# UCD4IDS/WaveletsExt.jl

Hardware: AMD Instinct MI355X
Metric: Msamples/s (fwd+inv wavelet packets) (higher is better)
Workload: dtype f64

## Files before the change

### waveletsext.jl_amd/__init__.py

```python
from .filters import WT, OrthoFilter, ArgumentError, wavelet, daubechies
from .util import (maxtransformlevels, isdyadic, ndyadicscales, nodelength, getchildindex,
                   getparentindex, getdepth, gettreelength, maketree, isvalidtree, getleaf,
                   getrowrange, getcolrange, main2depthshift, coarsestscalingrange,
                   finestdetailrange, delete_subtree)
from ._arrays import jl_empty, to_device, to_numpy, to_colmajor
from ._lib import WxError, build_info, device_count, red2d_route, set_force_generic, set_host_hugepages, shutdown, LIB_PATH
from .dwt import (wpd, wpd_, wpdall, iwpd, iwpd_, iwpdall, wpt, wpt_, iwpt, iwpt_,
                  wptall, iwptall, getbasiscoef, getbasiscoefall, dwt, idwt, dwtall, idwtall)
from .swt import (sdwt, sdwt_, sdwtall, isdwt, isdwt_, isdwtall, swpt, swpt_, swptall, iswpt, iswpt_,
                  iswptall, swpd, swpd_, swpdall, iswpd, iswpd_, iswpdall)
from .acwt import (acdwt, acdwt_, acdwtall, iacdwt, iacdwt_, iacdwtall, acwpt, acwpt_, acwptall,
                   iacwpt, iacwpt_, iacwptall, acwpd, acwpd_, acwpdall, iacwpd, iacwpd_, iacwpdall,
                   autocorr, pfilter, qfilter, make_acqmfpair, make_acreverseqmfpair)
from .bestbasis import (JBB, LoglpCost, NormCost, tree_costs, bestbasistree, bestbasis_treeselection,
                        jbb_moments, costs_from_moments, acwpd_jbb_moments,
                        BB, ShannonEntropyCost, LogEnergyEntropyCost, bestbasistreeall,
                        LSDB, DifferentialEntropyCost, lsdb_entropy)
from .denoising import (HardTH, SoftTH, SemiSoftTH, SteinTH, VisuShrink, SureShrink, RelErrorShrink,
                        noisest, threshold, denoise, denoiseall, surethreshold, relerrorthreshold,
                        surethresholdall, relerrorthresholdall)
from .ldb import (TimeFrequency, AsymmetricRelativeEntropy, SymmetricRelativeEntropy, LpDistance,
                  HellingerDistance, EarthMoverDistance, ProbabilityDensity, Signatures, SignatureMap, BasisDiscriminantMeasure,
                  FishersClassSeparability, RobustFishersClassSeparability, energy_map,
                  discriminant_measure, discriminant_power, LocalDiscriminantBasis, fit_, fitdec_, transform,
                  fit_transform, inverse_transform, change_nfeatures)
from .siwt import (ShiftInvariantWaveletTransformNode, ShiftInvariantWaveletTransformObject,
                   ShiftInvariantWaveletTransformBatch, siwpd, siwpdall, isiwpd, isiwpdall, bestbasistree_,
                   bestbasistreeall_, delete_node_)
from . import siwt as _siwt
_isvalidtree_arrays = isvalidtree


def isvalidtree(*args, **kw):
    if len(args) == 1 and isinstance(args[0], ShiftInvariantWaveletTransformObject):
        return _siwt.isvalidtree(args[0], **kw)
    return _isvalidtree_arrays(*args, **kw)
```

### waveletsext.jl_amd/_lib.py

```python
import ctypes
import os

_HERE = os.path.dirname(os.path.abspath(__file__))
LIB_PATH = os.environ.get("WX_HIP_LIB") or os.path.join(_HERE, "csrc", "libwaveletsext_hip.so")

WX_OK, WX_EASSERT, WX_EARG, WX_EBOUNDS, WX_EHIP, WX_EUNSUPPORTED = 0, -1, -2, -3, -10, -11


class WxError(RuntimeError):
    def __init__(self, code, msg):
        super().__init__("libwaveletsext_hip status %d: %s" % (code, msg))
        self.code = code


_lib = None


def lib():
    global _lib
    if _lib is None:
        if not os.path.exists(LIB_PATH):
            raise ImportError(
                "libwaveletsext_hip.so is not built (%s). Run `python -c 'import __graft_entry__ as g; "
                "g.build()'` or `make -C waveletsext.jl_amd/csrc`. There is no CPU fallback." % LIB_PATH)
# ... 97 lines not shown
    "wx_class_median_mad_f64": [_P, _L, _L, _P, _I, _P, _P, _P],
    "wx_class_median_mad_f32": [_P, _L, _L, _P, _I, _P, _P, _P],
    "wx_emd_measure_f64": [_P, _L, _L, _P, _I, _P, _P],
    "wx_emd_measure_f32": [_P, _L, _L, _P, _I, _P, _P],
    "wx_pdf_energy_map_f64": [_P, _L, _L, _P, _I, _P, _P],
    "wx_pdf_energy_map_f32": [_P, _L, _L, _P, _I, _P, _P],
    "wx_signature_weights_f64": [_P, _L, _L, _P, _I, _P, _P],
    "wx_signature_weights_f32": [_P, _L, _L, _P, _I, _P, _P],
    "wx_emd_measure_weighted_f64": [_P, _P, _L, _L, _P, _I, _P, _P],
    "wx_emd_measure_weighted_f32": [_P, _P, _L, _L, _P, _I, _P, _P],
    "wx_noisest_f64": [_P, _L, _L, _L, _L, _L, _P, _P],
    "wx_noisest_f32": [_P, _L, _L, _L, _L, _L, _P, _P],
    "wx_threshold_f64": [_P, _P, _L, _L, _L, _I, _P, _L, _L, _P, _P],
    "wx_threshold_f32": [_P, _P, _L, _L, _L, _I, _P, _L, _L, _P, _P],
    "wx_dwt3d_f64": [_P, _P, _L, _L, _L, _I, _L, _P, _I, _P],
    "wx_dwt3d_f32": [_P, _P, _L, _L, _L, _I, _L, _P, _I, _P],
    "wx_idwt3d_f64": [_P, _P, _L, _L, _L, _I, _L, _P, _I, _P],
    "wx_idwt3d_f32": [_P, _P, _L, _L, _L, _I, _L, _P, _I, _P],
    "wx_denoiseall_dwt_f64": [_P, _P, _L, _I, _L, _P, _I, _I, ctypes.c_double, _I, _P, _P],
    "wx_denoiseall_dwt_f32": [_P, _P, _L, _I, _L, _P, _I, _I, ctypes.c_double, _I, _P, _P],
    "wx_denoiseall_sig_f64": [_P, _P, _L, _I, _L, _P, _I, _I, ctypes.c_double, _I, _P, _P],
    "wx_denoiseall_sig_f32": [_P, _P, _L, _I, _L, _P, _I, _I, ctypes.c_double, _I, _P, _P],
    "wx_iwpt1d_thresh_f64": [_P, _P, _L, _I, _P, _L, _L, _P, _I, _I, _P, _L, _L, ctypes.c_double, _P],
    "wx_iwpt1d_thresh_f32": [_P, _P, _L, _I, _P, _L, _L, _P, _I, _I, _P, _L, _L, ctypes.c_double, _P],
    "wx_surethreshold_f64": [_P, _L, _L, _L, _P, _P, _P],
    "wx_surethreshold_f32": [_P, _L, _L, _L, _P, _P, _P],
    "wx_relerrorthreshold_f64": [_P, _L, _L, _L, _P, _I, _P, _P],
    "wx_relerrorthreshold_f32": [_P, _L, _L, _L, _P, _I, _P, _P],
    "wx_bb_costs_f64": [_P, _P, _L, _L, _L, _I, _I, _P],
    "wx_bb_costs_f32": [_P, _P, _L, _L, _L, _I, _I, _P],
    "wx_bb_costs2d_f64": [_P, _P, _L, _L, _L, _L, _I, _I, _P],
    "wx_bb_costs2d_f32": [_P, _P, _L, _L, _L, _L, _I, _I, _P],
    "wx_lsdb_entropy_f64": [_P, _L, _L, _P, _P],
    "wx_lsdb_entropy_f32": [_P, _L, _L, _P, _P],
    "wx_lsdb_costs_f64": [_P, _L, _L, _L, _I, _P, _P],
    "wx_lsdb_costs_f32": [_P, _L, _L, _L, _I, _P, _P],
    "wx_lsdb_costs2d_f64": [_P, _L, _L, _L, _L, _I, _P, _P],
    "wx_lsdb_costs2d_f32": [_P, _L, _L, _L, _L, _I, _P, _P],
    "wx_treeselect_batch_f64": [_P, _L, _L, _L, _I, _L, _P, _P],
    "wx_treeselect_batch_f32": [_P, _L, _L, _L, _I, _L, _P, _P],
    "wx_comm_unique_id": [_P],
    "wx_comm_init": [_I, _I, _P, ctypes.POINTER(ctypes.c_void_p)],
    "wx_comm_destroy": [_P],
    "wx_allgather_out_f64": [_P, _P, _L, _P, _P],
    "wx_allgather_out_f32": [_P, _P, _L, _P, _P],
    "wx_allgatherv_out_f64": [_P, _P, _P, _I, _P, _P],
    "wx_allgatherv_out_f32": [_P, _P, _P, _I, _P, _P],
    "wx_allreduce_moments_f64": [_P, _L, _P, _P],
    "wx_allreduce_moments_f32": [_P, _L, _P, _P],
}


def check(rc):
    if rc == WX_OK:
        return
    msg = lib().wx_last_error().decode("utf-8", "replace")
    if rc == WX_EASSERT:
        raise AssertionError(msg)
    if rc == WX_EARG:
        from .filters import ArgumentError
        raise ArgumentError(msg)
    if rc == WX_EBOUNDS:
        raise IndexError(msg)
    raise WxError(rc, msg)


def device_count():
    return lib().wx_device_count()


def build_info():
    return lib().wx_build_info().decode("utf-8", "replace")


def shutdown():
    check(lib().wx_shutdown())


def set_host_hugepages(on):
    return bool(lib().wx_set_host_hugepages(1 if on else 0))


def set_force_generic(on):
    lib().wx_debug_set_dispatch(2 if on == 2 else (1 if on else 0))


RED2D_ROUTES = {1: "F1", 2: "F2", 3: "F3", 4: "I1", 5: "I2", 6: "I3", 7: "I4"}


def red2d_route(inverse, m, n, L, elem_size, F, ac=False, shift=False):
    code = lib().wx_debug_red2d_route(int(bool(inverse)), m, n, L, elem_size, F, int(bool(ac)), int(bool(shift)))
    if code < 0:
        raise ValueError("wx_debug_red2d_route: arguments outside the transforms' domain")
    return RED2D_ROUTES[code & 255], code >> 8
```

### waveletsext.jl_amd/csrc/wx_api.hip

```cpp
#include "../../include/waveletsext_hip.h"
#include "wx_host.h"
#include "wx_debug.h"
#include "wx_kernels.h"
#include "wx_lanetree.h"
#include "wx_lattice_dn_api.h"
#include <atomic>
#include <cstring>

const char *wx_err_cstr();
static std::atomic<int> g_force_generic{0};
int wx_force_generic() { return g_force_generic.load() == 1; }
int wx_skip_register_kernels() { return g_force_generic.load() == 2; }

extern "C" {

int wx_version(void) { return 100;  }
const char *wx_last_error(void) { return wx_err_cstr(); }
int wx_device_count(void)
{
    int n = 0;
    if (hipGetDeviceCount(&n) != hipSuccess) { (void)hipGetLastError(); return 0; }
    return n;
}
void wx_debug_set_dispatch(int on) { g_force_generic.store(on == 2 ? 2 : (on ? 1 : 0)); }

}

#define WX_REQUIRE(cond, code, msg) \
    do { if (!(cond)) return wx_set_error(code, msg); } while (0)

static int wx_need_device()
{
    if (wx_device_count() < 1) return wx_set_error(WX_EHIP, "no HIP device visible: the MI355X kernels cannot run");
    return WX_OK;
}

template <typename T>
static int api_wpd1d(const T *x, T *y, int64_t n, int L, int64_t batch, const double *qmf, int F, void *stream)
{
    WxFilt filt;
    int rc = wx_pack_filter(qmf, F, &filt);
    if (rc) return rc;
    WX_REQUIRE(n >= 1 && batch >= 0, WX_EARG, "wpd: bad dimensions");
    WX_REQUIRE(0 <= L && L <= wx_maxtransformlevels(n), WX_EASSERT, "wpd!: 0 <= L <= maxtransformlevels(x) (DWT.jl:137)");
    WX_REQUIRE(n < ((int64_t)1 << 30), WX_EUNSUPPORTED, "wpd: signal length >= 2^30 not supported");
    if ((rc = wx_need_device())) return rc;
    hipStream_t st = wx_stream(stream);
    WxIO io(st);
    const T *dx = (const T *)io.in(x, sizeof(T) * n * batch);
    T *dy = (T *)io.out(y, sizeof(T) * n * (L + 1) * batch);
    if ((batch && n) && (!dx || !dy)) return io.finish(WX_EHIP);
    rc = wx_dev_wpd1d<T>(dx, dy, n, L, batch, filt, st, wx_force_generic());
    return io.finish(rc);
}

struct WxTree1d {
    int Leff = 0;
    const uint8_t *dstatus = nullptr;
    int64_t nstatus = 0;
    bool full = true;
};

static int wx_resolve_tree1d(int64_t n, int L, const uint8_t *tree, int64_t ntree, WxScratch &scr, WxTree1d *out,
                             const char *who)
{
    (void)who;
    WX_REQUIRE(wx_isdyadic(n), WX_EASSERT, "maketree/isvalidtree: signal length must be dyadic (Wavelets.jl)");
    if (!tree) {
        WX_REQUIRE(0 <= L && L <= wx_maxtransformlevels(n), WX_EASSERT, "maketree: 0 <= L <= maxtransformlevels(n)");
        out->Leff = L;
        out->full = true;
        return WX_OK;
    }
    WX_REQUIRE(wx_isvalidtree1d(n, tree, ntree), WX_EASSERT, "@assert isvalidtree(x, tree)");
    out->Leff = wx_tree_depth1d(tree, ntree);
    bool full = true;
    for (int64_t i = 1; i <= ((int64_t)1 << out->Leff) - 1 && full; ++i) full = tree[i - 1] != 0;
    out->full = full;
    if (!full) {
        out->dstatus = (const uint8_t *)scr.upload(tree, (size_t)ntree);
        if (!out->dstatus) return WX_EHIP;
        out->nstatus = ntree;
    }
    return WX_OK;
}

template <typename T>
static int wx_pyramid_tail(int64_t n, int F, bool inverse, const uint8_t *tree, int64_t ntree, std::vector<uint8_t> &cut, const WxFilt &filt,
                           bool allow_long = false)
{
    if (!tree || wx_force_generic()) return 0;
    const int Ld = wx_tree_depth1d(tree, ntree);
    bool pyramid = Ld >= 1;
    for (int64_t i = 1; i <= ntree && pyramid; ++i) pyramid = (tree[i - 1] != 0) == ((i & (i - 1)) == 0 && i < ((int64_t)1 << Ld));
    if (!pyramid) return 0;
    const int tail = wx_dwt_tail_levels(n, Ld, F, sizeof(T));
    if (!tail || (inverse && !((wx_fused1d_ok<T>(n, F) || (allow_long && wx_dwt_long_ok<T>(n, filt))) && Ld - tail >= 2))) return 0;
    cut.assign(tree, tree + ntree);
    for (int64_t i = (int64_t)1 << (Ld - tail); i <= ntree; ++i) cut[i - 1] = 0;
    return tail;
}

template <typename T, bool INVERSE>
static int api_wpt1d(const T *x, T *y, int64_t n, int L, const uint8_t *tree, int64_t ntree, int64_t batch,
                     const double *qmf, int F, void *stream)
{
    WxFilt filt;
// ... 368 lines not shown
```

### waveletsext.jl_amd/csrc/wx_debug.h

```cpp
#pragma once
#include <stdint.h>
#ifdef __cplusplus
extern "C" {
#endif
void wx_debug_set_dispatch(int mode);

int wx_debug_red2d_route(int inverse, int64_t m, int64_t n, int L, int elem_size, int F, int ac, int shift);
#ifdef __cplusplus
}
#endif
```

### waveletsext.jl_amd/csrc/wx_lattice.hip

```cpp
#include "wx_lattice_dev.h"

bool wx_lattice_factor(const WxFilt &filt, int L, bool inverse, WxLat *out)
{
    const int F = filt.F;
    if (F < 2 || (F & 1) || F / 2 > WX_LAT_MAXS) return false;
    const int J = F / 2 - 1;
    long double G[WX_LAT_MAXS][2][2] = {};
    for (int m = 0; m <= J; ++m) {
        G[m][0][0] = filt.q[2 * m];
        G[m][0][1] = filt.q[2 * m + 1];
        G[J - m][1][0] = -(long double)filt.q[2 * m + 1];
        G[J - m][1][1] = filt.q[2 * m];
    }
    long double t[WX_LAT_MAXS], cs[WX_LAT_MAXS];
    for (int deg = J; deg >= 1; --deg) {
        const int k = (fabsl(G[deg][0][0]) + fabsl(G[deg][1][0]) >= fabsl(G[deg][0][1]) + fabsl(G[deg][1][1])) ? 0 : 1;
        const long double a0 = G[deg][0][k], a1 = G[deg][1][k], r = hypotl(a0, a1);
        if (!(r > 0)) return false;
        const long double c = a1 / r, s = a0 / r;
        long double Hm[WX_LAT_MAXS][2][2];
        for (int m = 0; m <= deg; ++m)
            for (int col = 0; col < 2; ++col) {
                Hm[m][0][col] = c * G[m][0][col] - s * G[m][1][col];
                Hm[m][1][col] = s * G[m][0][col] + c * G[m][1][col];
            }
        for (int col = 0; col < 2; ++col)
            if (fabsl(Hm[deg][0][col]) > 1e-13L || fabsl(Hm[0][1][col]) > 1e-13L) return false;
        for (int m = 0; m < deg; ++m)
            for (int col = 0; col < 2; ++col) {
                G[m][0][col] = Hm[m][0][col];
                G[m][1][col] = Hm[m + 1][1][col];
            }
        if (fabsl(c) < 1e-3L) return false;
        t[deg] = s / c;
        cs[deg] = c;
    }
    {
        const long double c = G[0][0][0], s = G[0][0][1];
        if (fabsl(G[0][1][0] + s) > 1e-13L || fabsl(G[0][1][1] - c) > 1e-13L || fabsl(c) < 1e-3L) return false;
        t[0] = s / c;
        cs[0] = c;
    }
    long double gain1 = 1;
    double tr[WX_LAT_MAXS];
    for (int j = 0; j <= J; ++j) {
        tr[j] = (double)t[j];
        gain1 *= cs[j];
    }
    long double P[WX_LAT_MAXS][2][2] = {};
    P[0][0][0] = 1; P[0][0][1] = tr[0]; P[0][1][0] = -(long double)tr[0]; P[0][1][1] = 1;
    for (int j = 1; j <= J; ++j) {
        long double Q[WX_LAT_MAXS][2][2] = {};
        const long double tj = tr[j];
        for (int m = 0; m < j; ++m)
            for (int col = 0; col < 2; ++col) {
                Q[m][0][col] += P[m][0][col];
                Q[m + 1][0][col] += tj * P[m][1][col];
                Q[m][1][col] += -tj * P[m][0][col];
                Q[m + 1][1][col] += P[m][1][col];
            }
        for (int m = 0; m <= j; ++m)
            for (int r2 = 0; r2 < 2; ++r2)
                for (int col = 0; col < 2; ++col) P[m][r2][col] = Q[m][r2][col];
    }
    for (int m = 0; m <= J; ++m)
        if (fabsl(gain1 * P[m][0][0] - filt.q[2 * m]) > 1e-14L || fabsl(gain1 * P[m][0][1] - filt.q[2 * m + 1]) > 1e-14L)
            return false;
    long double sig = 1;
    for (int j = 0; j < WX_LAT_MAXS; ++j) {
        if (j <= J) {
            const long double c2 = 1 / (1 + t[j] * t[j]);
            out->p[j] = (double)(t[j] / sig);
            out->kap[j] = (double)(sig * t[j] * c2);
            sig *= c2;
        } else {
            out->p[j] = out->kap[j] = 0.0;
        }
    }
    const long double gL = powl(gain1, L);
    out->g0 = (double)(inverse ? 1 / gL : gL);
    out->g2 = (double)(inverse ? gain1 * gain1 : 1 / (gain1 * gain1));
    return std::isfinite(out->g0) && fabsl(gL) > 1e-60L && fabsl(gL) < 1e60L;
}

bool wx_lattice_coeffs(const WxFilt &filt, int L, bool inverse, double *p, double *kap, double *g0, double *g2)
{
    WxLat c;
    if (!wx_lattice_factor(filt, L, inverse, &c)) return false;
    for (int j = 0; j < WX_LAT_MAXS; ++j) { p[j] = c.p[j]; kap[j] = c.kap[j]; }
    *g0 = c.g0;
    *g2 = c.g2;
    return true;
}

int wx_lattice_launch_sh(bool inverse, const double *x, double *y, int64_t n, int L, int64_t batch, int64_t in_stride,
                         const WxFilt &filt, hipStream_t st);
int wx_lattice_launch_g(bool inverse, const double *x, double *y, int64_t n, int L, int64_t batch, int64_t in_stride,
                        const WxFilt &filt, hipStream_t st);
int wx_lattice_wpd_g_f64(const double *x, double *y, int64_t n, int L, int64_t batch, const WxFilt &filt, hipStream_t st);
int wx_lattice_launch_lo(bool inverse, const double *x, double *y, int L, int64_t batch, int64_t in_stride, const WxFilt &filt,
                         hipStream_t st);

static int wx_lattice_launch(bool inverse, const double *x, double *y, int64_t n, int L, int64_t batch, int64_t in_stride,
                             const WxFilt &filt, hipStream_t st)
{
    if (n == 2048 || n == 1024)
        return wx_lattice_launch_sh(inverse, x, y, n, L, batch, inverse ? in_stride : n, filt, st);
    if (n >= 64 && n <= 512)
        return wx_lattice_launch_g(inverse, x, y, n, L, batch, inverse ? in_stride : n, filt, st);
    if (n == 4096 && L >= 1 && L <= 5) return wx_lattice_launch_lo(inverse, x, y, L, batch, inverse ? in_stride : n, filt, st);
    if (n != 4096 || L < 6 || L > 12 || filt.F < 2 || batch <= 0) return 0;
    if ((reinterpret_cast<uintptr_t>(x) | reinterpret_cast<uintptr_t>(y)) & 31) return 0;
    if (inverse && (in_stride & 3)) return 0;
    WxLat cf;
    if (!wx_lattice_factor(filt, L, inverse, &cf)) return 0;
    int64_t grid = batch;
    if (grid > 0x7fffffff) grid = 0x7fffffff;
#define WX_GO(NSS)                                                                                                  \
    case NSS:                                                                                                       \
        if (inverse)                                                                                                \
            hipLaunchKernelGGL((k_lat_iwpt_f64<NSS, 2>), dim3((unsigned)grid), dim3(64), 0, st, x, y, L, batch, in_stride, cf); \
        else                                                                                                        \
            hipLaunchKernelGGL((k_lat_wpt_f64<NSS, 3>), dim3((unsigned)grid), dim3(64), 0, st, x, y, L, batch, cf);  \
        break;
    switch (wx_lat_stages(filt.F)) {
        WX_GO(1) WX_GO(2) WX_GO(4) WX_GO(6) WX_GO(8) WX_GO(10)
    default: return 0;
    }
#undef WX_GO
    const hipError_t e = hipGetLastError();
    if (e != hipSuccess) return wx_set_hip_error(e, "lattice wpt launch", __FILE__, __LINE__);
    return 1;
}

int wx_lattice_wpd_sh_f64(const double *x, double *y, int64_t n, int L, int64_t batch, const WxFilt &filt, hipStream_t st);

int wx_lattice_wpd_f64(const double *x, double *y, int64_t n, int L, int64_t batch, const WxFilt &filt, hipStream_t st)
{
    if ((n == 2048 || n == 1024) && x != (const double *)y) return wx_lattice_wpd_sh_f64(x, y, n, L, batch, filt, st);
    if (n >= 64 && n <= 512 && x != (const double *)y) return wx_lattice_wpd_g_f64(x, y, n, L, batch, filt, st);
    if (n != 4096 || L < 1 || L > 12 || filt.F < 2 || batch <= 0 || batch > 0x7fffffff) return 0;
    if ((reinterpret_cast<uintptr_t>(x) | reinterpret_cast<uintptr_t>(y)) & 31) return 0;
    WxLatW cw;
    if (!wx_lattice_factor(filt, L, false, &cw.c)) return 0;
    {
        const long double g2 = cw.c.g2;
        long double g = 1 / sqrtl(g2);
        WxLat tmp;
        if (!wx_lattice_factor(filt, 1, false, &tmp)) return 0;
        g = tmp.g0;
        long double acc = 1;
        for (int l = 0; l <= 12; ++l) { cw.gl[l] = (double)acc; acc *= g; }
    }
#define WX_GOW(NSS)                                                                                                 \
    case NSS:                                                                                                       \
        hipLaunchKernelGGL((k_lat_wpd_f64<NSS, 2>), dim3((unsigned)batch), dim3(64), 0, st, x, y, L, batch, cw);     \
        break;
    switch (wx_lat_stages(filt.F)) {
        WX_GOW(1) WX_GOW(2) WX_GOW(4) WX_GOW(6) WX_GOW(8) WX_GOW(10)
    default: return 0;
    }
#undef WX_GOW
    const hipError_t e = hipGetLastError();
    if (e != hipSuccess) return wx_set_hip_error(e, "lattice wpd launch", __FILE__, __LINE__);
    return 1;
}

bool wx_lattice_applicable_f64(const WxFilt &filt)
{
    if (filt.F < 2 || filt.F / 2 > WX_LAT_MAXS) return false;
    WxLat tmp;
    return wx_lattice_factor(filt, 6, false, &tmp);
}

int wx_lattice_wpt8k_f64(const double *x, double *y, int L, int64_t batch, const WxFilt &filt, hipStream_t st);
int wx_lattice_iwpt8k_f64(const double *xw, double *y, int L, int64_t batch, int64_t in_stride, const WxFilt &filt, hipStream_t st);

int wx_lattice_wpt_f64(const double *x, double *y, int64_t n, int L, int64_t batch, const WxFilt &filt, hipStream_t st)
{
    if (n == 8192) return wx_lattice_wpt8k_f64(x, y, L, batch, filt, st);
    return wx_lattice_launch(false, x, y, n, L, batch, n, filt, st);
}
int wx_lattice_iwpt_f64(const double *xw, double *y, int64_t n, int L, int64_t batch, int64_t in_stride, const WxFilt &filt,
                        hipStream_t st)
{
    if (n == 8192) return wx_lattice_iwpt8k_f64(xw, y, L, batch, in_stride, filt, st);
    return wx_lattice_launch(true, xw, y, n, L, batch, in_stride, filt, st);
}

#define WX_TREE_DECL(k)                                                                                              \
    int wx_lattice_tree##k##_f64(bool, const double *, double *, int64_t, int, int64_t, int64_t, int64_t, const WxFilt &, \
                                 const uint8_t *, int64_t, const WxThreshArg *, hipStream_t, int64_t);
WX_TREE_DECL(0f) WX_TREE_DECL(0i) WX_TREE_DECL(1f) WX_TREE_DECL(1i) WX_TREE_DECL(2f) WX_TREE_DECL(2i)
#undef WX_TREE_DECL

#define WX_TREES_DECL(k)                                                                                                             \
    int wx_lattice_trees_##k##_f64(const double *, double *, int64_t, int, int64_t, int64_t, int64_t, const WxFilt &, const uint8_t *, int64_t, hipStream_t, int64_t); \
    int wx_lattice_trees_##k##_f32(const float *, float *, int64_t, int, int64_t, int64_t, int64_t, const WxFilt &, const uint8_t *, int64_t, hipStream_t, int64_t);
WX_TREES_DECL(3f) WX_TREES_DECL(3i) WX_TREES_DECL(4f) WX_TREES_DECL(4i) WX_TREES_DECL(5f) WX_TREES_DECL(5i) WX_TREES_DECL(6f) WX_TREES_DECL(6i)
#undef WX_TREES_DECL
// ... 63 lines not shown
```

### waveletsext.jl_amd/csrc/wx_lattice_8ki.hip

```cpp
#include "wx_lattice_8k.h"
bool wx_lattice_factor(const WxFilt &filt, int L, bool inverse, WxLat *out);
int wx_lattice_iwpt8k_f64(const double *xw, double *y, int L, int64_t batch, int64_t in_stride, const WxFilt &filt, hipStream_t st)
{
    if (L < 7 || L > 13 || filt.F < 2 || filt.F > 20 || batch <= 0 || batch > 0x7fffffff || xw == y) return 0;
    if ((reinterpret_cast<uintptr_t>(xw) | reinterpret_cast<uintptr_t>(y)) & 31) return 0;
    if (in_stride < 8192 || (in_stride & 3)) return 0;
    WxLat cf;
    if (!wx_lattice_factor(filt, L - 1, true, &cf)) return 0;
#define WX_GO8(NSS)                                                                                                      \
    case NSS: hipLaunchKernelGGL((k_lat_iwpt8k_f64<NSS, 2>), dim3((unsigned)batch), dim3(128), 0, st, xw, y, L - 1, batch, in_stride, cf, filt); break;
    switch (wx_lat_stages(filt.F)) {
        WX_GO8(1) WX_GO8(2) WX_GO8(4) WX_GO8(6) WX_GO8(8) WX_GO8(10)
    default: return 0;
    }
#undef WX_GO8
    const hipError_t e = hipGetLastError();
    if (e != hipSuccess) return wx_set_hip_error(e, "lattice iwpt launch (8192 samples)", __FILE__, __LINE__);
    return 1;
}
```

### waveletsext.jl_amd/csrc/wx_lattice_dev.h

```cpp
#pragma once
#include "wx_common.h"
#include "wx_kernels.h"
#include <cmath>
#include <cstdlib>
#include <utility>

#define WX_LAT_MAXS 10
#define WX_LAT_LDS 1104

struct WxLat {
    double p[WX_LAT_MAXS];
    double kap[WX_LAT_MAXS];
    double g0;
    double g2;
};

namespace {

__device__ __forceinline__ void lat_sync()
{
    __builtin_amdgcn_fence(__ATOMIC_RELEASE, "wavefront");
    __builtin_amdgcn_wave_barrier();
    __builtin_amdgcn_fence(__ATOMIC_ACQUIRE, "wavefront");
}
// ... 1011 lines not shown
    lat_level<3, 0, NS, false>(c, cf);
    lat_emit<6, 10>(c, lds0, ys + 4096 * 10, lane, cw);
    if (L < 11) return;
    lat_level<4, 0, NS, false>(c, cf);
    lat_emit<6, 11>(c, lds0, ys + 4096 * 11, lane, cw);
    if (L < 12) return;
    lat_level<5, 0, NS, false>(c, cf);
    lat_emit<6, 12>(c, lds0, ys + 4096 * 12, lane, cw);
}

__device__ __forceinline__ double lat_ld1(const double __attribute__((address_space(1))) *p) { return *p; }
template <int SH> constexpr int lat_rotr(int p) { return (p >> SH) | ((p & ((1 << SH) - 1)) << (12 - SH)); }

template <int NS, int WPE, int SH>
__global__ __launch_bounds__(64) __attribute__((amdgpu_waves_per_eu(WPE, WPE))) void k_lat_wpt_sh_f64(
    const double *__restrict__ x, double *__restrict__ y, int L, int last_sig, WxLatW cw)
{
    static_assert(SH == 1 || SH == 2, "two or four signals per wavefront");
    __shared__ double lds[WX_LAT_LDS];
    const unsigned lds0 = (unsigned)(uintptr_t)(double __attribute__((address_space(3))) *)lds;
    const int lane = threadIdx.x;
    const int sig0 = min((int)blockIdx.x << SH, last_sig);
    const int64_t off = (int64_t)sig0 * (4096 >> SH);
    const double *xs = x + off;
    double *ys = y + off;
    const WxLat &cf = cw.c;
    double a[64];
    {
        lat_d2 r[32];
        const int lp = 64 * (lane >> 3) + 2 * (lane & 7);
        const unsigned xo = (unsigned)((lp >> SH) | ((lp & ((1 << SH) - 1)) << (12 - SH)));
        lat_for<32>([&](auto Q) {
            constexpr int hi3 = Q / 4, f = Q % 4;
            r[Q].x = lat_ld1(lat_sbase(xs + lat_rotr<SH>(512 * hi3 + 16 * f)) + xo);
            r[Q].y = lat_ld1(lat_sbase(xs + lat_rotr<SH>(512 * hi3 + 16 * f + 1)) + xo);
        });
        const unsigned wa = lds0 + 8u * (17u * (lane >> 3) + 2u * (lane & 7)), ra = lds0 + 8u * 17u * lane;
        lat_for<4>([&](auto Fq) {
            constexpr int f = Fq;
            lat_for<8>([&](auto Hq) {
                constexpr int hi3 = Hq;
                lds_wr<8 * (136 * hi3)>(wa, r[4 * hi3 + f].x);
                lds_wr<8 * (136 * hi3 + 1)>(wa, r[4 * hi3 + f].y);
            });
            double t[16];
            lat_for<16>([&](auto M) {
                constexpr int m = M;
                t[m] = lds_rd<8 * m>(ra);
            });
            lat_wait16<0>(t);
            lat_for<16>([&](auto M) {
                constexpr int m = M;
                a[16 * f + m] = t[m];
            });
        });
    }
    if constexpr (SH < 2) lat_level<1, 6, NS, false>(a, cf);
    double bb[64];
    lat_t2(a, bb, lds0, lane);
    lat_level<0, 4, NS, false>(bb, cf);
    lat_level<1, 4, NS, false>(bb, cf);
    lat_level<2, 4, NS, false>(bb, cf);
    lat_level<3, 4, NS, false>(bb, cf);
    double c[64];
    lat_t3(bb, c, lds0, lane);
    const int Le = L + SH;
    if (Le > 6) lat_level<0, 0, NS, false>(c, cf);
    if (Le > 7) lat_level<1, 0, NS, false>(c, cf);
    if (Le > 8) lat_level<2, 0, NS, false>(c, cf);
    if (Le > 9) lat_level<3, 0, NS, false>(c, cf);
    if (Le > 10) lat_level<4, 0, NS, false>(c, cf);
    if (Le > 11) lat_level<5, 0, NS, false>(c, cf);
    switch (Le) {
    case 6: lat_emit<6, 6 - SH + 16 * SH>(c, lds0, ys, lane, cw); break;
    case 7: lat_emit<6, 7 - SH + 16 * SH>(c, lds0, ys, lane, cw); break;
    case 8: lat_emit<6, 8 - SH + 16 * SH>(c, lds0, ys, lane, cw); break;
    case 9: lat_emit<6, 9 - SH + 16 * SH>(c, lds0, ys, lane, cw); break;
    case 10: lat_emit<6, 10 - SH + 16 * SH>(c, lds0, ys, lane, cw); break;
    case 11: lat_emit<6, 11 - SH + 16 * SH>(c, lds0, ys, lane, cw); break;
    default: lat_emit<6, 12 - SH + 16 * SH>(c, lds0, ys, lane, cw); break;
    }
}

template <int NS, typename TM, typename SINK>
__device__ __forceinline__ void lat_inv_to_l0(const TM *__restrict__ xs, unsigned lds0, int lane, int L, const WxLat &cf, SINK &&sink)
{
    double c[64];
    switch (L) {
    case 6: lat_load_c<6>(c, lds0, xs, lane, cf); break;
    case 7: lat_load_c<7>(c, lds0, xs, lane, cf); break;
    case 8: lat_load_c<8>(c, lds0, xs, lane, cf); break;
    case 9: lat_load_c<9>(c, lds0, xs, lane, cf); break;
    case 10: lat_load_c<10>(c, lds0, xs, lane, cf); break;
    case 11: lat_load_c<11>(c, lds0, xs, lane, cf); break;
    default: lat_load_c<12>(c, lds0, xs, lane, cf); break;
    }
    if (L > 11) lat_level<5, 0, NS, true>(c, cf);
    if (L > 10) lat_level<4, 0, NS, true>(c, cf);
    if (L > 9) lat_level<3, 0, NS, true>(c, cf);
    if (L > 8) lat_level<2, 0, NS, true>(c, cf);
    if (L > 7) lat_level<1, 0, NS, true>(c, cf);
    if (L > 6) lat_level<0, 0, NS, true>(c, cf);
    double bb[64];
    {
        const unsigned wa = lds0 + 8u * (34 * (lane >> 1) + (lane & 1));
        const int H = lane & 15, p0 = (lane >> 4) & 1, p1 = lane >> 5;
        const unsigned ra = lds0 + 8u * (34 * p1 + 2 * H + p0);
        lat_for<4>([&](auto Fq) {
            constexpr int f = Fq;
            lat_for<16>([&](auto Hq) {
                constexpr int Hh = Hq;
                lds_wr<8 * 2 * Hh>(wa, c[4 * Hh + f]);
            });
            double t[16];
            lat_for<16>([&](auto Jq) {
                constexpr int j = Jq;
                t[j] = lds_rd<8 * 68 * j>(ra);
            });
            lat_wait16<0>(t);
            lat_for<16>([&](auto Jq) {
                constexpr int j = Jq;
                bb[16 * f + j] = t[j];
            });
        });
    }
    lat_level<3, 4, NS, true>(bb, cf);
    lat_level<2, 4, NS, true>(bb, cf);
    lat_level<1, 4, NS, true>(bb, cf);
    lat_level<0, 4, NS, true>(bb, cf);
    double a[64];
    {
        const int H = lane & 15, p10 = lane >> 4;
        unsigned wa[4];
#pragma unroll
        for (int h = 0; h < 4; ++h)
            wa[h] = lds0 + 8u * (((h ^ (H >> 2)) | ((H & 3) << 2) | (((H >> 2) & 1) << 4) | ((H >> 3) << 5)) + 64 * p10);
        const int Ha = lane >> 2, ha = lane & 3;
        const unsigned ra = lds0 + 8u * ((ha ^ (Ha >> 2)) | ((Ha & 3) << 2) | (((Ha >> 2) & 1) << 4) | ((Ha >> 3) << 5));
        lat_for<4>([&](auto Fq) {
            constexpr int f = Fq;
            lat_for<16>([&](auto Q) {
                constexpr int h = Q / 4, g = Q % 4;
                lds_wr<8 * 256 * g>(wa[h], bb[16 * h + 4 * f + g]);
            });
            double t[16];
            lat_for<16>([&](auto Jq) {
                constexpr int j = Jq;
                t[j] = lds_rd<8 * 64 * j>(ra);
            });
            lat_wait16<0>(t);
            lat_for<16>([&](auto Jq) {
                constexpr int j = Jq;
                a[16 * f + j] = t[j];
            });
        });
    }
    lat_level<1, 6, NS, true>(a, cf);
    lat_level<0, 6, NS, true>(a, cf);
    lat_t1i(a, lds0, lane, sink);
}

template <int NS, int WPE, typename TM = double>
__global__ __launch_bounds__(64) __attribute__((amdgpu_waves_per_eu(WPE, WPE))) void k_lat_iwpt_f64(
    const TM *__restrict__ xw, TM *__restrict__ y, int L, int64_t batch, int64_t in_stride, WxLat cf)
{
    __shared__ double lds[WX_LAT_LDS];
    const unsigned lds0 = (unsigned)(uintptr_t)(double __attribute__((address_space(3))) *)lds;
    const int lane = threadIdx.x;
    const int64_t sig = blockIdx.x;
    const unsigned yo = 64u * (lane >> 3) + 2u * (lane & 7);
    TM *ys = y + sig * 4096;
    lat_inv_to_l0<NS>(xw + sig * in_stride, lds0, lane, L, cf, [&](auto Fq, lat_d2 (&o)[8]) {
        constexpr int f = decltype(Fq)::value;
        lat_for<8>([&](auto Hq) {
            constexpr int hi3 = Hq;
            lat_st2(lat_sbase(ys + 512 * hi3 + 16 * f) + yo, o[hi3]);
        });
    });
}

template <int NS, int WPE, int SH>
__global__ __launch_bounds__(64) __attribute__((amdgpu_waves_per_eu(WPE, WPE))) void k_lat_wpd_sh_f64(
    const double *__restrict__ x, double *__restrict__ y, int L, int last_sig, WxLatW cw)
{
    static_assert(SH == 1 || SH == 2, "two or four signals per wavefront");
    __shared__ double lds[WX_LAT_LDS];
    const unsigned lds0 = (unsigned)(uintptr_t)(double __attribute__((address_space(3))) *)lds;
    const int lane = threadIdx.x;
    constexpr int N = 4096 >> SH;
    const int sig0 = min((int)blockIdx.x << SH, last_sig);
    const double *xs = x + (int64_t)sig0 * N;
    const unsigned ts = (unsigned)(N * (L + 1));
    double *ys = y + (int64_t)sig0 * ts;
    const WxLat &cf = cw.c;
    double a[64];
    {
        lat_d2 r[32];
        const int lp = 64 * (lane >> 3) + 2 * (lane & 7);
        const unsigned xo = (unsigned)((lp >> SH) | ((lp & ((1 << SH) - 1)) << (12 - SH)));
        lat_for<32>([&](auto Q) {
            constexpr int hi3 = Q / 4, f = Q % 4;
            r[Q].x = lat_ld1(lat_sbase(xs + lat_rotr<SH>(512 * hi3 + 16 * f)) + xo);
            r[Q].y = lat_ld1(lat_sbase(xs + lat_rotr<SH>(512 * hi3 + 16 * f + 1)) + xo);
        });
        const unsigned wa = lds0 + 8u * (17u * (lane >> 3) + 2u * (lane & 7)), ra = lds0 + 8u * 17u * lane;
        lat_for<4>([&](auto Fq) {
            constexpr int f = Fq;
            lat_for<8>([&](auto Hq) {
                constexpr int hi3 = Hq;
                lds_wr<8 * (136 * hi3)>(wa, r[4 * hi3 + f].x);
                lds_wr<8 * (136 * hi3 + 1)>(wa, r[4 * hi3 + f].y);
            });
            double t[16];
            lat_for<16>([&](auto M) {
                constexpr int m = M;
                t[m] = lds_rd<8 * m>(ra);
            });
            lat_wait16<0>(t);
            lat_for<16>([&](auto M) {
                constexpr int m = M;
                a[16 * f + m] = t[m];
            });
        });
    }
    lat_emit<0, 16 * SH>(a, lds0, ys, lane, cw, ts);
#define WX_LVL_A(K)                                                                               \
    if constexpr (K >= SH) {                                                                      \
        constexpr int l = K - SH + 1;                                                             \
        lat_level<K, 6, NS, false>(a, cf);                                                        \
        lat_emit<0, l + 16 * SH>(a, lds0, ys + N * l, lane, cw, ts);                              \
        if (L <= l) return;                                                                       \
    }
    WX_LVL_A(1)
#undef WX_LVL_A
    double bb[64];
    lat_t2(a, bb, lds0, lane);
#define WX_LVL_B(K)                                                                               \
    {                                                                                             \
        constexpr int l = K + 2 - SH + 1;                                                         \
        lat_level<K, 4, NS, false>(bb, cf);                                                       \
        lat_emit<2, l + 16 * SH>(bb, lds0, ys + N * l, lane, cw, ts);                             \
        if (L <= l) return;                                                                       \
// ... 407 lines not shown
```

Before: 39610.

## Fold top inverse lattice levels into a dense per-node matrix for L=12

For the inverse wavelet packet lattice at depth 12 (and 13 in the 8192-sample kernel), the host now precomputes a small dense matrix (8x8 or 4x4) that combines the top two or three inverse lattice levels. The kernel applies that matrix to the register-resident coefficients with FMAs instead of running several sequential lattice stages with shifts. This cuts the serial dependency chain and per-stage overhead, but adds NF multiply-adds per output and passes a larger kernel argument. Numerical behaviour changes slightly, and a debug dispatch mode is added to turn the fold off.

```diff
diff --git a/waveletsext.jl_amd/__init__.py b/waveletsext.jl_amd/__init__.py
--- a/waveletsext.jl_amd/__init__.py
+++ b/waveletsext.jl_amd/__init__.py
@@ -4,7 +4,7 @@
                    getrowrange, getcolrange, main2depthshift, coarsestscalingrange,
                    finestdetailrange, delete_subtree)
 from ._arrays import jl_empty, to_device, to_numpy, to_colmajor
-from ._lib import WxError, build_info, device_count, red2d_route, set_force_generic, set_host_hugepages, shutdown, LIB_PATH
+from ._lib import WxError, build_info, device_count, lattice_fold_matrix, red2d_route, set_force_generic, set_host_hugepages, shutdown, LIB_PATH
 from .dwt import (wpd, wpd_, wpdall, iwpd, iwpd_, iwpdall, wpt, wpt_, iwpt, iwpt_,
                   wptall, iwptall, getbasiscoef, getbasiscoefall, dwt, idwt, dwtall, idwtall)
 from .swt import (sdwt, sdwt_, sdwtall, isdwt, isdwt_, isdwtall, swpt, swpt_, swptall, iswpt, iswpt_,
diff --git a/waveletsext.jl_amd/_lib.py b/waveletsext.jl_amd/_lib.py
--- a/waveletsext.jl_amd/_lib.py
+++ b/waveletsext.jl_amd/_lib.py
@@ -203,7 +203,18 @@
 
 
 def set_force_generic(on):
-    lib().wx_debug_set_dispatch(2 if on == 2 else (1 if on else 0))
+    lib().wx_debug_set_dispatch(on if on in (2, 3) else (1 if on else 0))
+
+
+def lattice_fold_matrix(qmf, nf, inverse=True):
+    import numpy as np
+    q = np.ascontiguousarray(qmf, dtype=np.float64)
+    m = np.zeros((nf, nf), dtype=np.float64)
+    f = lib().wx_debug_lattice_fold
+    f.argtypes = [_P, _I, _I, _I, _P]
+    f.restype = _I
+    got = f(q.ctypes.data, int(q.size), int(nf), 1 if inverse else 0, m.ctypes.data)
+    return m if got == nf else None
 
 
 RED2D_ROUTES = {1: "F1", 2: "F2", 3: "F3", 4: "I1", 5: "I2", 6: "I3", 7: "I4"}
diff --git a/waveletsext.jl_amd/csrc/wx_api.hip b/waveletsext.jl_amd/csrc/wx_api.hip
--- a/waveletsext.jl_amd/csrc/wx_api.hip
+++ b/waveletsext.jl_amd/csrc/wx_api.hip
@@ -11,6 +11,7 @@
 static std::atomic<int> g_force_generic{0};
 int wx_force_generic() { return g_force_generic.load() == 1; }
 int wx_skip_register_kernels() { return g_force_generic.load() == 2; }
+int wx_lattice_no_fold() { return g_force_generic.load() == 3; }
 
 extern "C" {
 
@@ -22,7 +23,7 @@
     if (hipGetDeviceCount(&n) != hipSuccess) { (void)hipGetLastError(); return 0; }
     return n;
 }
-void wx_debug_set_dispatch(int on) { g_force_generic.store(on == 2 ? 2 : (on ? 1 : 0)); }
+void wx_debug_set_dispatch(int on) { g_force_generic.store((on == 2 || on == 3) ? on : (on ? 1 : 0)); }
 
 }
 
diff --git a/waveletsext.jl_amd/csrc/wx_debug.h b/waveletsext.jl_amd/csrc/wx_debug.h
--- a/waveletsext.jl_amd/csrc/wx_debug.h
+++ b/waveletsext.jl_amd/csrc/wx_debug.h
@@ -5,6 +5,8 @@
 #endif
 void wx_debug_set_dispatch(int mode);
 
+int wx_debug_lattice_fold(const double *q, int F, int NF, int inverse, double *m);
+
 int wx_debug_red2d_route(int inverse, int64_t m, int64_t n, int L, int elem_size, int F, int ac, int shift);
 #ifdef __cplusplus
 }
diff --git a/waveletsext.jl_amd/csrc/wx_lattice.hip b/waveletsext.jl_amd/csrc/wx_lattice.hip
--- a/waveletsext.jl_amd/csrc/wx_lattice.hip
+++ b/waveletsext.jl_amd/csrc/wx_lattice.hip
@@ -1,4 +1,4 @@
-#include "wx_lattice_dev.h"
+#include "wx_lattice_fold.h"
 
 bool wx_lattice_factor(const WxFilt &filt, int L, bool inverse, WxLat *out)
 {
@@ -83,6 +83,58 @@
     return std::isfinite(out->g0) && fabsl(gL) > 1e-60L && fabsl(gL) < 1e60L;
 }
 
+bool wx_lattice_fold_matrix(const WxLat &cf, int NS, int NF, bool inverse, double *m)
+{
+    if (NS < 1 || NS > WX_LAT_MAXS || (NF != 2 && NF != 4 && NF != 8)) return false;
+    const int nb = NF == 2 ? 1 : (NF == 4 ? 2 : 3);
+    for (int col = 0; col < NF; ++col) {
+        long double x[8] = {};
+        x[col] = 1;
+        for (int k = 0; k < nb; ++k) {
+            const int b = inverse ? nb - 1 - k : k, S = 1 << b, M = NF >> (b + 1);
+            for (int s = 0; s < S; ++s) {
+                long double u[4], w[4], old[4];
+                for (int mm = 0; mm < M; ++mm) { u[mm] = x[s + ((2 * mm) << b)]; w[mm] = x[s + ((2 * mm) << b) + S]; }
+                auto shift = [&](int sh) {
+                    for (int mm = 0; mm < M; ++mm) old[mm] = w[mm];
+                    for (int mm = 0; mm < M; ++mm) w[mm] = old[(((mm + sh) % M) + M) % M];
+                };
+                if (!inverse) {
+                    for (int j = 0; j < NS; ++j) {
+                        for (int mm = 0; mm < M; ++mm) { u[mm] += (long double)cf.p[j] * w[mm]; w[mm] -= (long double)cf.kap[j] * u[mm]; }
+                        if (j + 1 < NS) shift(1);
+                    }
+                    shift(-(NS - 1));
+                } else {
+                    shift(NS - 1);
+                    for (int j = NS - 1; j >= 0; --j) {
+                        for (int mm = 0; mm < M; ++mm) { w[mm] += (long double)cf.kap[j] * u[mm]; u[mm] -= (long double)cf.p[j] * w[mm]; }
+                        if (j > 0) shift(-1);
+                    }
+                }
+                for (int mm = 0; mm < M; ++mm) { x[s + ((2 * mm) << b)] = u[mm]; x[s + ((2 * mm) << b) + S] = w[mm]; }
+            }
+        }
+        for (int i = 0; i < NF; ++i) {
+            if (!std::isfinite((double)x[i]) || fabsl(x[i]) > 1e30L) return false;
+            m[NF * i + col] = (double)x[i];
+        }
+    }
+    return true;
+}
+
+extern "C" int wx_debug_lattice_fold(const double *q, int F, int NF, int inverse, double *m)
+{
+    if (!q || !m || F < 2 || F > WX_MAXF) return 0;
+    WxFilt filt = {};
+    for (int i = 0; i < F; ++i) filt.q[i] = q[i];
+    filt.F = F;
+    WxLat cf;
+    const int NS = wx_lat_stages(F);
+    if (NS < 6 || NS > WX_LAT_MAXS || !wx_lattice_factor(filt, 12, inverse != 0, &cf)) return 0;
+    return wx_lattice_fold_matrix(cf, NS, NF, inverse != 0, m) ? NF : 0;
+}
+
 bool wx_lattice_coeffs(const WxFilt &filt, int L, bool inverse, double *p, double *kap, double *g0, double *g2)
 {
     WxLat c;
@@ -116,6 +168,19 @@
     if (!wx_lattice_factor(filt, L, inverse, &cf)) return 0;
     int64_t grid = batch;
     if (grid > 0x7fffffff) grid = 0x7fffffff;
+    if (inverse && L == 12 && wx_lat_stages(filt.F) >= 6 && !wx_lattice_no_fold()) {
+        WxLatFold<WX_LAT_FOLD> fm;
+        if (wx_lattice_fold_matrix(cf, wx_lat_stages(filt.F), WX_LAT_FOLD, true, fm.m)) {
+            switch (wx_lat_stages(filt.F)) {
+            case 6: hipLaunchKernelGGL((k_lat_iwpt12_f64<6, 2, WX_LAT_FOLD>), dim3((unsigned)grid), dim3(64), 0, st, x, y, batch, in_stride, cf, fm); break;
+            case 8: hipLaunchKernelGGL((k_lat_iwpt12_f64<8, 2, WX_LAT_FOLD>), dim3((unsigned)grid), dim3(64), 0, st, x, y, batch, in_stride, cf, fm); break;
+            default: hipLaunchKernelGGL((k_lat_iwpt12_f64<10, 2, WX_LAT_FOLD>), dim3((unsigned)grid), dim3(64), 0, st, x, y, batch, in_stride, cf, fm); break;
+            }
+            const hipError_t ef = hipGetLastError();
+            if (ef != hipSuccess) return wx_set_hip_error(ef, "lattice iwpt launch (folded)", __FILE__, __LINE__);
+            return 1;
+        }
+    }
 #define WX_GO(NSS)                                                                                                  \
     case NSS:                                                                                                       \
         if (inverse)                                                                                                \
diff --git a/waveletsext.jl_amd/csrc/wx_lattice_8ki.hip b/waveletsext.jl_amd/csrc/wx_lattice_8ki.hip
--- a/waveletsext.jl_amd/csrc/wx_lattice_8ki.hip
+++ b/waveletsext.jl_amd/csrc/wx_lattice_8ki.hip
@@ -1,5 +1,25 @@
 #include "wx_lattice_8k.h"
+#include "wx_lattice_fold.h"
 bool wx_lattice_factor(const WxFilt &filt, int L, bool inverse, WxLat *out);
+
+namespace {
+template <int NS, int WPE, int NF>
+__global__ __launch_bounds__(128) __attribute__((amdgpu_waves_per_eu(WPE, WPE))) void k_lat_iwpt8k12_f64(
+    const double *__restrict__ xw, double *__restrict__ y, int64_t batch, int64_t in_stride, WxLat cf, WxFilt filt, WxLatFold<NF> fm)
+{
+    __shared__ double lds2[2][WX_LAT_LDS];
+    __shared__ __attribute__((aligned(16))) double xch[2][2][512 + 16];
+    const int child = __builtin_amdgcn_readfirstlane((int)(threadIdx.x >> 6)), lane = threadIdx.x & 63;
+    const unsigned lds0 = (unsigned)(uintptr_t)(double __attribute__((address_space(3))) *)lds2[child];
+    const int64_t sig = blockIdx.x;
+    lat_d2 o[32];
+    lat_inv12_to_l0<NS, NF>(xw + sig * in_stride + 4096 * child, lds0, lane, cf, fm, [&](auto Fq, lat_d2 (&oo)[8]) {
+        constexpr int f = decltype(Fq)::value;
+        lat_for<8>([&](auto Hq) { o[4 * Hq + f] = oo[Hq]; });
+    });
+    lat8k_synth<2 * NS>(o, xch, child, lane, y + sig * 8192, filt);
+}
+}
 int wx_lattice_iwpt8k_f64(const double *xw, double *y, int L, int64_t batch, int64_t in_stride, const WxFilt &filt, hipStream_t st)
 {
     if (L < 7 || L > 13 || filt.F < 2 || filt.F > 20 || batch <= 0 || batch > 0x7fffffff || xw == y) return 0;
@@ -7,6 +27,19 @@
     if (in_stride < 8192 || (in_stride & 3)) return 0;
     WxLat cf;
     if (!wx_lattice_factor(filt, L - 1, true, &cf)) return 0;
+    if (L == 13 && wx_lat_stages(filt.F) >= 6 && !wx_lattice_no_fold()) {
+        WxLatFold<4> fm;
+        if (wx_lattice_fold_matrix(cf, wx_lat_stages(filt.F), 4, true, fm.m)) {
+            switch (wx_lat_stages(filt.F)) {
+            case 6: hipLaunchKernelGGL((k_lat_iwpt8k12_f64<6, 2, 4>), dim3((unsigned)batch), dim3(128), 0, st, xw, y, batch, in_stride, cf, filt, fm); break;
+            case 8: hipLaunchKernelGGL((k_lat_iwpt8k12_f64<8, 2, 4>), dim3((unsigned)batch), dim3(128), 0, st, xw, y, batch, in_stride, cf, filt, fm); break;
+            default: hipLaunchKernelGGL((k_lat_iwpt8k12_f64<10, 2, 4>), dim3((unsigned)batch), dim3(128), 0, st, xw, y, batch, in_stride, cf, filt, fm); break;
+            }
+            const hipError_t ef = hipGetLastError();
+            if (ef != hipSuccess) return wx_set_hip_error(ef, "lattice iwpt launch (8192 samples, folded)", __FILE__, __LINE__);
+            return 1;
+        }
+    }
 #define WX_GO8(NSS)                                                                                                      \
     case NSS: hipLaunchKernelGGL((k_lat_iwpt8k_f64<NSS, 2>), dim3((unsigned)batch), dim3(128), 0, st, xw, y, L - 1, batch, in_stride, cf, filt); break;
     switch (wx_lat_stages(filt.F)) {
diff --git a/waveletsext.jl_amd/csrc/wx_lattice_dev.h b/waveletsext.jl_amd/csrc/wx_lattice_dev.h
--- a/waveletsext.jl_amd/csrc/wx_lattice_dev.h
+++ b/waveletsext.jl_amd/csrc/wx_lattice_dev.h
@@ -1117,25 +1117,9 @@
     }
 }
 
-template <int NS, typename TM, typename SINK>
-__device__ __forceinline__ void lat_inv_to_l0(const TM *__restrict__ xs, unsigned lds0, int lane, int L, const WxLat &cf, SINK &&sink)
-{
-    double c[64];
-    switch (L) {
-    case 6: lat_load_c<6>(c, lds0, xs, lane, cf); break;
-    case 7: lat_load_c<7>(c, lds0, xs, lane, cf); break;
-    case 8: lat_load_c<8>(c, lds0, xs, lane, cf); break;
-    case 9: lat_load_c<9>(c, lds0, xs, lane, cf); break;
-    case 10: lat_load_c<10>(c, lds0, xs, lane, cf); break;
-    case 11: lat_load_c<11>(c, lds0, xs, lane, cf); break;
-    default: lat_load_c<12>(c, lds0, xs, lane, cf); break;
-    }
-    if (L > 11) lat_level<5, 0, NS, true>(c, cf);
-    if (L > 10) lat_level<4, 0, NS, true>(c, cf);
-    if (L > 9) lat_level<3, 0, NS, true>(c, cf);
-    if (L > 8) lat_level<2, 0, NS, true>(c, cf);
-    if (L > 7) lat_level<1, 0, NS, true>(c, cf);
-    if (L > 6) lat_level<0, 0, NS, true>(c, cf);
+template <int NS, typename SINK>
+__device__ __forceinline__ void lat_inv_c_to_l0(double (&c)[64], unsigned lds0, int lane, const WxLat &cf, SINK &&sink)
+{
     double bb[64];
     {
         const unsigned wa = lds0 + 8u * (34 * (lane >> 1) + (lane & 1));
@@ -1193,6 +1177,28 @@
     lat_level<1, 6, NS, true>(a, cf);
     lat_level<0, 6, NS, true>(a, cf);
     lat_t1i(a, lds0, lane, sink);
+}
+
+template <int NS, typename TM, typename SINK>
+__device__ __forceinline__ void lat_inv_to_l0(const TM *__restrict__ xs, unsigned lds0, int lane, int L, const WxLat &cf, SINK &&sink)
+{
+    double c[64];
+    switch (L) {
+    case 6: lat_load_c<6>(c, lds0, xs, lane, cf); break;
+    case 7: lat_load_c<7>(c, lds0, xs, lane, cf); break;
+    case 8: lat_load_c<8>(c, lds0, xs, lane, cf); break;
+    case 9: lat_load_c<9>(c, lds0, xs, lane, cf); break;
+    case 10: lat_load_c<10>(c, lds0, xs, lane, cf); break;
+    case 11: lat_load_c<11>(c, lds0, xs, lane, cf); break;
+    default: lat_load_c<12>(c, lds0, xs, lane, cf); break;
+    }
+    if (L > 11) lat_level<5, 0, NS, true>(c, cf);
+    if (L > 10) lat_level<4, 0, NS, true>(c, cf);
+    if (L > 9) lat_level<3, 0, NS, true>(c, cf);
+    if (L > 8) lat_level<2, 0, NS, true>(c, cf);
+    if (L > 7) lat_level<1, 0, NS, true>(c, cf);
+    if (L > 6) lat_level<0, 0, NS, true>(c, cf);
+    lat_inv_c_to_l0<NS>(c, lds0, lane, cf, sink);
 }
 
 template <int NS, int WPE, typename TM = double>
diff --git a/waveletsext.jl_amd/csrc/wx_lattice_fold.h b/waveletsext.jl_amd/csrc/wx_lattice_fold.h
--- /dev/null
+++ b/waveletsext.jl_amd/csrc/wx_lattice_fold.h
@@ -0,0 +1,82 @@
+#pragma once
+#include "wx_lattice_dev.h"
+
+#ifndef WX_LAT_FOLD
+#define WX_LAT_FOLD 8
+#endif
+
+template <int NF> struct WxLatFold {
+    double m[NF * NF];
+};
+
+bool wx_lattice_fold_matrix(const WxLat &cf, int NS, int NF, bool inverse, double *m);
+int wx_lattice_no_fold();
+
+namespace {
+
+template <int NF> __device__ __forceinline__ void lat_fold_nodes(double (&c)[64], const WxLatFold<NF> &fm)
+{
+    constexpr int G = 64 / NF, RB = NF < 4 ? NF : 4, NB = NF / RB;
+    double t[NB > 1 ? (NB - 1) * G * RB : 1];
+    lat_for<NB>([&](auto Bc) {
+        constexpr int b = Bc;
+        lat_for<G>([&](auto Sc) {
+            constexpr int s = Sc;
+            double o[RB];
+            lat_for<RB>([&](auto Ic) {
+                constexpr int row = RB * b + Ic;
+                double acc = fm.m[NF * row] * c[s];
+                lat_for<NF - 1>([&](auto Jc) {
+                    constexpr int j = Jc + 1;
+                    acc = fma(fm.m[NF * row + j], c[s + G * j], acc);
+                });
+                o[Ic] = acc;
+            });
+            if constexpr (b + 1 < NB) {
+                lat_for<RB>([&](auto Ic) { t[(b * G + s) * RB + Ic] = o[Ic]; });
+            } else {
+                lat_for<NB - 1>([&](auto Pc) {
+                    lat_for<RB>([&](auto Ic) { c[s + G * (RB * Pc + Ic)] = t[(Pc * G + s) * RB + Ic]; });
+                });
+                lat_for<RB>([&](auto Ic) { c[s + G * (RB * b + Ic)] = o[Ic]; });
+            }
+        });
+    });
+}
+
+template <int NS, int NF, typename TM, typename SINK>
+__device__ __forceinline__ void lat_inv12_to_l0(const TM *__restrict__ xs, unsigned lds0, int lane, const WxLat &cf,
+                                                const WxLatFold<NF> &fm, SINK &&sink)
+{
+    static_assert(NF == 2 || NF == 4 || NF == 8, "levels 12, 11 + 12, 10 + 11 + 12");
+    double c[64];
+    lat_load_c<12>(c, lds0, xs, lane, cf);
+    lat_fold_nodes<NF>(c, fm);
+    if constexpr (NF < 4) lat_level<4, 0, NS, true>(c, cf);
+    if constexpr (NF < 8) lat_level<3, 0, NS, true>(c, cf);
+    lat_level<2, 0, NS, true>(c, cf);
+    lat_level<1, 0, NS, true>(c, cf);
+    lat_level<0, 0, NS, true>(c, cf);
+    lat_inv_c_to_l0<NS>(c, lds0, lane, cf, sink);
+}
+
+template <int NS, int WPE, int NF>
+__global__ __launch_bounds__(64) __attribute__((amdgpu_waves_per_eu(WPE, WPE))) void k_lat_iwpt12_f64(
+    const double *__restrict__ xw, double *__restrict__ y, int64_t batch, int64_t in_stride, WxLat cf, WxLatFold<NF> fm)
+{
+    __shared__ double lds[WX_LAT_LDS];
+    const unsigned lds0 = (unsigned)(uintptr_t)(double __attribute__((address_space(3))) *)lds;
+    const int lane = threadIdx.x;
+    const int64_t sig = blockIdx.x;
+    const unsigned yo = 64u * (lane >> 3) + 2u * (lane & 7);
+    double *ys = y + sig * 4096;
+    lat_inv12_to_l0<NS, NF>(xw + sig * in_stride, lds0, lane, cf, fm, [&](auto Fq, lat_d2 (&o)[8]) {
+        constexpr int f = decltype(Fq)::value;
+        lat_for<8>([&](auto Hq) {
+            constexpr int hi3 = Hq;
+            lat_st2(lat_sbase(ys + 512 * hi3 + 16 * f) + yo, o[hi3]);
+        });
+    });
+}
+
+}
```

Result: no change. 40200 (median of 6 runs) (+1.5%).
